# mlvlab/UP-NeRF

Hardware: AMD Instinct MI355X
Metric: training rays/sec (higher is better)
Workload: dtype f32 (f16x3 emulated: 3 fp16 MFMAs per product, fp32 accumulate); 1 GPU; BASELINE.json configs[1]: Brandenburg Gate shape, 4096 rays/GPU/step, 64 coarse + 128 fine samples, two 8x256 fields + candidate/colour heads + TransientNet + appearance/candidate embeddings (763 images), pose optimisation ON, full step incl. both Adam updates; rays_per_gpu=4096, n_images=763, N_samples=64, N_importance=128, parallelism=dp1, field=f16x3

## Files before the change

### include/upnerf_hip.h

```cpp
#ifndef UPNERF_HIP_H
#define UPNERF_HIP_H

#include <stdint.h>

#ifdef __cplusplus
extern "C" {
#endif

#define UPNERF_ABI_VERSION 11
#define UPNERF_EINVAL (-1)
#define UPNERF_EUNSUP (-2)

#ifndef UPNERF_TILE_ROWS
#define UPNERF_TILE_ROWS 64
#endif
#define UPNERF_X0 64
#define UPNERF_AUXK 80
#define UPNERF_CK 16
#define UPNERF_MAX_D 8

int upnerf_abi_version(void);

int upnerf_pose_rays_fwd(int R, const float* se3, const float* c2w, const float* dirs,
                         float* rays_o, float* rays_d, void* stream);
// ... 275 lines not shown
  int32_t planes;
  upnerf_wgrad_operand A, B;
  const int32_t* expo_a; const int32_t* expo_b;
  float* dW; float* db;
  int32_t ldo;
  int32_t n2;
  float* dW2; float* db2;
  int32_t ldo2, nsplit;
  const float* v; float* dv; float* dbv;
  float* slabs;
} upnerf_wgrad_desc;
long long upnerf_wgrad16_scratch(const upnerf_wgrad_desc* d);
int upnerf_wgrad16(const upnerf_wgrad_desc* d, upnerf_wgrad_pending* pending, void* stream);
int upnerf_wgrad_finish(upnerf_wgrad_pending* pending, void* stream);

int upnerf_vec_wgrad(int M, const float* v, int ldv, int nvec, const float* X, int ldx, int K,
                     float* dw , float* dbv , float* scratch, int nsplit, void* stream);

int upnerf_vec_wgrad_frag16(int M, const float* v, int ldv, int nvec, const uint16_t* X16, const int32_t* xexp, int K, float* dw,
                            float* dbv, float* scratch, int nsplit, void* stream);

int upnerf_ray_sum(int R, int S, const float* X, int C, float* out, void* stream);
int upnerf_ray_geom_bwd(int R, int S, const float* dxyz, const float* z, float* d_o, float* d_d, void* stream);

typedef struct {
  int32_t R, h, C;
  const int64_t* idx;
  const float* all_ray_infos;
  const float* all_directions;
  const float* all_rgbs;
// ... 539 lines not shown
```

### upnerf_amd/_lib.py

```python
from __future__ import annotations

import ctypes as C
import os

import torch

from .pass_plan import (AUXK, CK, RR_PART_STRIDE, TILE_PART_STRIDE, WG_F16_FRAG, WG_F16_TILE, WG_F24, WG_F32,
                        WG_PLANES, X0)

_HERE = os.path.dirname(os.path.abspath(__file__))
LIB_PATH = os.environ.get("UPNERF_LIB") or os.path.join(_HERE, "libupnerf_hip.so")
MAX_D = 8

_fp = C.c_void_p


class Layout(C.Structure):
    _fields_ = [("W", C.c_int32), ("D", C.c_int32), ("skip", C.c_int32),
                ("w", C.c_int32 * MAX_D), ("b", C.c_int32 * MAX_D),
                ("we", C.c_int32), ("be", C.c_int32), ("wsig", C.c_int32), ("bsig", C.c_int32),
                ("wc1", C.c_int32), ("bc1", C.c_int32), ("wc2", C.c_int32), ("bc2", C.c_int32),
                ("wcsig", C.c_int32), ("bcsig", C.c_int32), ("wr1", C.c_int32), ("br1", C.c_int32),
                ("wr2", C.c_int32), ("br2", C.c_int32), ("total", C.c_int32),
                ("t_w", C.c_int32 * MAX_D), ("t_skipx", C.c_int32), ("t_we", C.c_int32), ("t_head", C.c_int32),
# ... 93 lines not shown

class WgradPending(C.Structure):
    _fields_ = [("slabs", _fp), ("bslabs", _fp), ("dW", _fp), ("db", _fp), ("N", C.c_int32), ("K", C.c_int32), ("TN", C.c_int32),
                ("TK", C.c_int32), ("nsplit", C.c_int32), ("ldo", C.c_int32), ("rblocks", C.c_int32), ("n2", C.c_int32),
                ("dW2", _fp), ("db2", _fp), ("ldo2", C.c_int32), ("pad", C.c_int32), ("vslabs", _fp), ("dv", _fp), ("dbv", _fp)]


class WgradOperand(C.Structure):
    _fields_ = [("p", _fp), ("lo", _fp), ("exp", _fp), ("ld", C.c_int32), ("kind", C.c_int32)]


class WgradDesc(C.Structure):
    _fields_ = [("M", C.c_int32), ("N", C.c_int32), ("K", C.c_int32), ("planes", C.c_int32), ("A", WgradOperand), ("B", WgradOperand),
                ("expo_a", _fp), ("expo_b", _fp), ("dW", _fp), ("db", _fp), ("ldo", C.c_int32), ("n2", C.c_int32), ("dW2", _fp),
                ("db2", _fp), ("ldo2", C.c_int32), ("nsplit", C.c_int32), ("v", _fp), ("dv", _fp), ("dbv", _fp), ("slabs", _fp)]


class WgradGroup(C.Structure):
    _fields_ = [("A", _fp), ("B", _fp), ("dW", _fp), ("db", _fp), ("M", C.c_int32), ("N", C.c_int32), ("K", C.c_int32),
                ("lda", C.c_int32), ("ldb", C.c_int32), ("ldo", C.c_int32)]


MAX_WGRAD_GROUPS = 32


class EmbedGroup(C.Structure):
    _fields_ = [("g", _fp), ("out", _fp), ("dim", C.c_int32)]


class EmbedRowsGroup(C.Structure):
# ... 255 lines not shown
    "upnerf_sort_rows": [_i, _i, _p, _p],
    "upnerf_sample_coarse_keyed": [_i, _i, _p, _p, C.POINTER(Rng), _f, _i, _p, _p],
    "upnerf_resample_sort": [_i, _i, _p, _p, _i, _i, _p, _i, _p, _i, _i, _p, _i, _i, C.POINTER(Rng), _p, _p],
    "upnerf_ray_aux": [_i, _p, _p, C.POINTER(C.c_float), _p, _p, _p],
    "upnerf_field_fwd": [C.POINTER(Layout), C.POINTER(FieldFwdArgs), _p],
    "upnerf_composite_fwd": [C.POINTER(CompositeFwdArgs), _p],
    "upnerf_composite_bwd": [C.POINTER(CompositeBwdArgs), _p],
    "upnerf_field_bwd": [C.POINTER(Layout), C.POINTER(FieldBwdArgs), _p],
    "upnerf_field_fwd_f16x3": [C.POINTER(Layout), C.POINTER(FieldFwdArgs), _p],
    "upnerf_field_bwd_f16x3": [C.POINTER(Layout), C.POINTER(FieldBwdArgs), _p],
    "upnerf_frag16": [_p, _p, _p, C.POINTER(Frag16Desc), _i, C.POINTER(Frag16Desc), _i, _p, _p, _i, _i, _p, _p],
    "upnerf_wgrad": [_i, _p, _i, _i, _p, _i, _i, _p, _i, _p, _p, _i, _p],
    "upnerf_wgrad16_scratch": [C.POINTER(WgradDesc)],
    "upnerf_wgrad16": [C.POINTER(WgradDesc), C.POINTER(WgradPending), _p],
    "upnerf_wgrad_finish": [_p, _p],
    "upnerf_transient_fwd": [_p, _p],
    "upnerf_transient_bwd": [_p, _p, _p],
    "upnerf_wgrad_grouped_scratch": [C.POINTER(WgradGroup), _i, _i],
    "upnerf_wgrad_grouped": [C.POINTER(WgradGroup), _i, _p, _i, _p],
    "upnerf_vec_wgrad": [_i, _p, _i, _i, _p, _i, _i, _p, _p, _p, _i, _p],
    "upnerf_matvec": [_i, _i, _p, _i, _p, _p, _p, _i, _p],
    "upnerf_matvec_rank1": [_i, _i, _p, _i, _p, _p, _p, _i, _p, _p],
    "upnerf_add_pairs": [C.POINTER(AddPair), _i, _p],
    "upnerf_zero": [_p, C.c_longlong, _p],
    "upnerf_vec_wgrad_frag16": [_i, _p, _i, _i, _p, _p, _i, _p, _p, _p, _i, _p],
    "upnerf_ray_sum": [_i, _i, _p, _i, _p, _p],
    "upnerf_ray_part_finish": [_i, _i, _p, _p, _p, _p],
    "upnerf_tile_part_finish": [_i, _i, _p, _p, _p, _p, _p, _p, _p, _p, _p],
    "upnerf_ray_geom_bwd": [_i, _i, _p, _p, _p, _p, _p],
    "upnerf_pack": [_p, C.POINTER(PackDesc), _i, _i, _p],
# ... 48 lines not shown
    "upnerf_vit_embed": [_i, _i, _p, _p, _p, _p],
    "upnerf_layernorm": [_i, _i, _p, _i, _p, _p, _f, _p, _i, _p],
    "upnerf_vit_attention": [C.POINTER(VitAttentionArgs), _p],
    "upnerf_vit_gelu": [_p, C.c_longlong, _p],
    "upnerf_vit_residual": [_p, _p, C.c_longlong, _p],
    "upnerf_pca_fit_scratch": [_i, _i],
    "upnerf_pca_fit": [C.POINTER(PcaFitArgs), _p, _p],
    "upnerf_conv3x3": [C.POINTER(Conv3x3Args), _p],
    "upnerf_upsample2x": [C.POINTER(Upsample2xArgs), _p],
    "upnerf_depth_to_space": [C.POINTER(DepthToSpaceArgs), _p],
    "upnerf_resize_cubic": [C.POINTER(ResizeCubicArgs), _p],
    "upnerf_vit_patches16": [C.POINTER(VitPatches16Args), _p],
    "upnerf_baked_render": [C.POINTER(BakedRenderArgs), _p],
    "upnerf_baked_pack": [C.POINTER(BakedPackArgs), _p],
}
_LONGLONG = ("upnerf_wgrad16_scratch", "upnerf_mtet_scratch", "upnerf_occ_words", "upnerf_occ_build_scratch",
             "upnerf_occ_compact_scratch", "upnerf_pca_fit_scratch")
MAX_SCALARS = 96
EXPORTS = tuple(_SIGNATURES)


def _load():
    if not os.path.exists(LIB_PATH):
        raise ImportError(
            f"{LIB_PATH} not found: the HIP extension is not built. Run `python __graft_entry__.py` "
            "(there is no CPU/PyTorch fallback for the render_rays hot path).")
    lib = C.CDLL(LIB_PATH)
    for name, argtypes in _SIGNATURES.items():
        fn = getattr(lib, name, None)
        if fn is None:
            raise ImportError(f"{LIB_PATH} does not export {name}; rebuild it")
# ... 39 lines not shown
```

### upnerf_amd/csrc/wgrad_f16x3.hip

```cpp
#include "common.cuh"
#include "wgrad_host.h"

namespace {

typedef _Float16 h8 __attribute__((ext_vector_type(8)));
typedef _Float16 h4 __attribute__((ext_vector_type(4)));
typedef short s4 __attribute__((ext_vector_type(4)));
typedef unsigned int u32x2_t __attribute__((ext_vector_type(2)));

#ifndef FX_CHUNK_BIG
#define FX_CHUNK_BIG 16
#endif

template <int FX_CHUNK>
__device__ __forceinline__ int himg(int row, int col) {
  const int panel = col >> 7, c = col & 127;
  return panel * (FX_CHUNK * 256) + 256 * row + 16 * ((c >> 3) ^ (((row & 3) << 2) | ((row >> 2) & 3))) + 2 * (c & 7);
}

__device__ __forceinline__ h4 tr_read(const char* base, int byteoff) {
  s4 v = __builtin_amdgcn_ds_read_tr16_b64_v4i16((s4 __attribute__((address_space(3)))*)(base + byteoff));
  return __builtin_bit_cast(h4, v);
}

#define FX_THREADS 512
#define WG_LOAD(p) NT_LOAD(p)
#define WG_OPLOAD(dst, p) dst = WG_LOAD((const f32x4*)(p))
#define WG_PIN_LOADS_P __builtin_amdgcn_sched_barrier(0)
template <int NP, int MTW, int NTW, bool HASV = false>
__global__ __launch_bounds__(FX_THREADS, 1) void wgrad_f16x3_kernel(int M, int N, int K, const float* __restrict__ A, int lda,
                                                                  const float* __restrict__ B, int ldb,
                                                                  const int* __restrict__ expo_a, const int* __restrict__ expo_b,
                                                                  float* __restrict__ slabs, float* __restrict__ bslabs,
                                                                  int rows_per_split, upnerf_wgrad_pending prev,
                                                                  const float* __restrict__ vrow = nullptr,
                                                                  float* __restrict__ vslabs = nullptr) {
  constexpr int TN = 64 * MTW, TK = 64 * NTW;
  constexpr int FX_CHUNK = (MTW * NTW == 16) ? FX_CHUNK_BIG : 32;
  constexpr int PN = (TN + 127) / 128, PK = (TK + 127) / 128;
  constexpr int SZA = PN * FX_CHUNK * 256, SZB = PK * FX_CHUNK * 256;
  constexpr int A4 = FX_CHUNK * TN / 4 / FX_THREADS, B4 = FX_CHUNK * TK / 4 / FX_THREADS;
  static_assert(A4 >= 1 && B4 >= 1, "tile too small for 512 threads");
  constexpr int WK = (TK >= 128) ? 4 : 2, WN = 8 / WK;
  constexpr int MT = (TN / WN >= 32) ? TN / WN / 32 : 1, NT = TK / WK / 32;
  constexpr bool HALF = TN / WN < 32;
  __shared__ __attribute__((aligned(16))) char lds[2 * (2 * SZA + 2 * SZB)];
  const int tid = threadIdx.x, lane = tid & 63, wave = tid >> 6;
  const int li = lane & 31, hh = lane >> 5;
  const bool active = !HALF || wave < 4;
  const int wn = HALF ? ((wave & 3) >> 1) : wave / WK, wk = HALF ? (wave & 1) : wave % WK;
  const int n0 = wn * 32 * MT, k0 = wk * 32 * NT;
  const int split = blockIdx.x;
  const int nblk = blockIdx.y * TN, kblk = blockIdx.z * TK;
  const int mbeg = split * rows_per_split;
  const int mend = (mbeg + rows_per_split < M) ? mbeg + rows_per_split : M;
  if (prev.nsplit > 0) {
    const int wg = (blockIdx.z * gridDim.y + blockIdx.y) * gridDim.x + blockIdx.x;
    if (wg < prev.rblocks) {
      wgrad_reduce_body(wg, tid, prev, (f32x4(*)[64])lds);
      __syncthreads();
    }
  }
  const int ea = expo_a[0], eb = expo_b[0];
  const float sa = ldexpf(1.0f, ea), sb = ldexpf(1.0f, eb);

  f32x16 acc[MT][NT];
  acc_zero(acc);
  f32x4 bsum = {0.f, 0.f, 0.f, 0.f};

  f32x4 ra0[A4], rb0[B4], ra1[A4], rb1[B4];
  float rv0[B4], rv1[B4];
  f32x4 vsum = {0.f, 0.f, 0.f, 0.f};
  float vtot = 0.0f;
  const int mlast = mend > mbeg ? mend - 1 : (mbeg < M ? mbeg : M - 1);
  auto gload = [&](f32x4 (&ra)[A4], f32x4 (&rb)[B4], float (&rv)[B4], int mc) {
#pragma unroll
    for (int q = 0; q < A4; ++q) {
      const int idx = tid + q * FX_THREADS, row = idx / (TN / 4), c4 = idx - row * (TN / 4);
      const int m = mc + row < mlast ? mc + row : mlast;
      const int col = nblk + 4 * c4 < N ? nblk + 4 * c4 : 0;
      WG_OPLOAD(ra[q], &A[(size_t)m * lda + col]);
    }
#pragma unroll
    for (int q = 0; q < B4; ++q) {
      const int idx = tid + q * FX_THREADS, row = idx / (TK / 4), c4 = idx - row * (TK / 4);
      const int m = mc + row < mlast ? mc + row : mlast;
      const int col = kblk + 4 * c4 < K ? kblk + 4 * c4 : 0;
      WG_OPLOAD(rb[q], &B[(size_t)m * ldb + col]);
      if constexpr (HASV) rv[q] = vrow[m];
    }
  };
  auto split_store = [&](char* hi, char* lo, f32x4 v, float s, int row, int col) {
    typedef float f2 __attribute__((ext_vector_type(2)));
    typedef _Float16 hh2 __attribute__((ext_vector_type(2)));
    const f2 x0 = f2{v[0], v[1]} * s, x1 = f2{v[2], v[3]} * s;
    const hh2 h0 = __builtin_convertvector(x0, hh2), h1 = __builtin_convertvector(x1, hh2);
    const int off = himg<FX_CHUNK>(row, col);
    *(h4*)(hi + off) = __builtin_shufflevector(h0, h1, 0, 1, 2, 3);
    if constexpr (NP == 2) {
      const hh2 l0 = __builtin_convertvector(x0 - __builtin_convertvector(h0, f2), hh2);
      const hh2 l1 = __builtin_convertvector(x1 - __builtin_convertvector(h1, f2), hh2);
      *(h4*)(lo + off) = __builtin_shufflevector(l0, l1, 0, 1, 2, 3);
    }
  };
  auto lstore = [&](const f32x4 (&ra)[A4], const f32x4 (&rb)[B4], const float (&rv)[B4], int buf, int mc) {
    char* base = lds + buf * (2 * SZA + 2 * SZB);
    const f32x4 z4 = {0.f, 0.f, 0.f, 0.f};
#pragma unroll
    for (int q = 0; q < A4; ++q) {
      const int idx = tid + q * FX_THREADS, row = idx / (TN / 4), c4 = idx - row * (TN / 4);
      const f32x4 v = (mc + row < mend && nblk + 4 * c4 < N) ? ra[q] : z4;
      bsum += v;
      split_store(base, base + SZA, v, sa, row, 4 * c4);
    }
#pragma unroll
    for (int q = 0; q < B4; ++q) {
      const int idx = tid + q * FX_THREADS, row = idx / (TK / 4), c4 = idx - row * (TK / 4);
      const f32x4 v = (mc + row < mend && kblk + 4 * c4 < K) ? rb[q] : z4;
      split_store(base + 2 * SZA, base + 2 * SZA + SZB, v, sb, row, 4 * c4);
      if constexpr (HASV) {
        const float vm = mc + row < mend ? rv[q] : 0.0f;
        vsum += v * vm;
        vtot += c4 == 0 ? vm : 0.0f;
      }
    }
  };
  const int g = lane >> 4, tq = (lane >> 2) & 3, tp = lane & 3;
  const int trow = 8 * (g >> 1) + tq, tcol = 16 * (g & 1) + 4 * tp;

  auto contract = [&](int buf) {
    if (!active) return;
    const char* base = lds + buf * (2 * SZA + 2 * SZB);
#pragma unroll
    for (int kk = 0; kk < FX_CHUNK / 16; ++kk) {
      h8 ah[MT], al[MT];
#pragma unroll
      for (int mt = 0; mt < MT; ++mt) {
        const int o0 = himg<FX_CHUNK>(16 * kk + trow, n0 + 32 * mt + tcol), o1 = himg<FX_CHUNK>(16 * kk + trow + 4, n0 + 32 * mt + tcol);
        const h4 x0 = tr_read(base, o0), x1 = tr_read(base, o1);
        ah[mt] = __builtin_shufflevector(x0, x1, 0, 1, 2, 3, 4, 5, 6, 7);
        if constexpr (NP == 2) {
          const h4 y0 = tr_read(base + SZA, o0), y1 = tr_read(base + SZA, o1);
          al[mt] = __builtin_shufflevector(y0, y1, 0, 1, 2, 3, 4, 5, 6, 7);
        }
// ... 7 lines not shown
        if constexpr (NP == 2) {
          const h4 y0 = tr_read(base + 2 * SZA + SZB, o0), y1 = tr_read(base + 2 * SZA + SZB, o1);
          bl = __builtin_shufflevector(y0, y1, 0, 1, 2, 3, 4, 5, 6, 7);
        }
#pragma unroll
        for (int mt = 0; mt < MT; ++mt) {
          acc[mt][nt] = __builtin_amdgcn_mfma_f32_32x32x16_f16(ah[mt], bh, acc[mt][nt], 0, 0, 0);
          if constexpr (NP == 2) {
            acc[mt][nt] = __builtin_amdgcn_mfma_f32_32x32x16_f16(ah[mt], bl, acc[mt][nt], 0, 0, 0);
            acc[mt][nt] = __builtin_amdgcn_mfma_f32_32x32x16_f16(al[mt], bh, acc[mt][nt], 0, 0, 0);
          }
        }
      }
    }
  };
  constexpr bool TWO_SETS = MT * NT * 16 <= 64 || FX_CHUNK == 16;
  if constexpr (TWO_SETS) {
    gload(ra0, rb0, rv0, mbeg);
    gload(ra1, rb1, rv1, mbeg + FX_CHUNK);
#pragma unroll 1
    for (int mc = mbeg; mc < mend; mc += 2 * FX_CHUNK) {
      lstore(ra0, rb0, rv0, 0, mc);
      __syncthreads();
      gload(ra0, rb0, rv0, mc + 2 * FX_CHUNK);
      contract(0);
      lstore(ra1, rb1, rv1, 1, mc + FX_CHUNK);
      __syncthreads();
      gload(ra1, rb1, rv1, mc + 3 * FX_CHUNK);
      contract(1);
    }
  } else {
    int buf = 0;
    gload(ra0, rb0, rv0, mbeg);
#pragma unroll 1
    for (int mc = mbeg; mc < mend; mc += FX_CHUNK) {
      lstore(ra0, rb0, rv0, buf, mc);
      __syncthreads();
      gload(ra0, rb0, rv0, mc + FX_CHUNK);
      contract(buf);
      buf ^= 1;
    }
  }
  const float unscale = ldexpf(1.0f, -(ea + eb));
  const size_t blk = ((size_t)split * gridDim.y + blockIdx.y) * gridDim.z + blockIdx.z;
  float* slab = slabs + blk * TN * TK;
  if (active) {
#pragma unroll
    for (int mt = 0; mt < MT; ++mt)
#pragma unroll
      for (int nt = 0; nt < NT; ++nt)
#pragma unroll
        for (int r = 0; r < 16; ++r) {
          const int n = n0 + 32 * mt + (r & 3) + 8 * (r >> 2) + 4 * hh;
          slab[n * TK + k0 + 32 * nt + li] = acc[mt][nt][r] * unscale;
        }
  }
  if (bslabs && blockIdx.z == 0) {
    __syncthreads();
    f32x4* red = (f32x4*)lds;
    red[tid] = bsum;
    __syncthreads();
    constexpr int Q = TN / 4, G = FX_THREADS / Q;
    if (tid < Q) {
      f32x4 s = red[tid];
#pragma unroll
      for (int j = 1; j < G; ++j) s += red[tid + j * Q];
      *(f32x4*)&bslabs[((size_t)split * gridDim.y + blockIdx.y) * TN + 4 * tid] = s;
    }
  }
  if constexpr (HASV) {
// ... 623 lines not shown
  upnerf_wgrad_pending P = reduce_desc(d->N, d->K, TN, TK, nsplit, d->slabs, L.bslabs, d->dW, d->ldo, d->db);
  P.n2 = d->n2;
  P.dW2 = d->dW2;
  P.db2 = d->db2;
  P.ldo2 = d->ldo2;
  P.vslabs = L.vslabs;
  P.dv = d->dv;
  P.dbv = d->dbv;
  if (pending) {
    *pending = P;
    return 0;
  }
  launch_reduce(L.st, P);
  return (int)hipGetLastError();
}
```

### upnerf_amd/ops.py

```python
from __future__ import annotations

import contextlib
import ctypes as C
import os
from typing import Dict, NamedTuple, Optional, Tuple

import torch
import torch.nn.functional as F

from . import _lib
from ._lib import check, lib, ptr, stream

_WS: Dict[Tuple[str, int], torch.Tensor] = {}


class KernelTimer:

    def __init__(self):
        self.enabled = False
        self.only = None
        self.records = {}

    def run(self, name: str, fn, units: int = 0):
        if not self.enabled or (self.only is not None and name not in self.only):
# ... 148 lines not shown
        p = self.t.data_ptr() + 4 * self.off if self.kind == _lib.WG_F32 else ptr(self.t)
        return _lib.WgradOperand(p=p, lo=ptr(self.lo), exp=ptr(self.exp), ld=self.ld, kind=self.kind)


_WG_TIMER = {_lib.WG_F32: "wgrad16", _lib.WG_F16_TILE: "wgrad16p", _lib.WG_F16_FRAG: "wgrad16p", _lib.WG_F24: "wgrad24p",
             _lib.WG_PLANES: "wgrad16hl"}


class WgradRun:

    def __init__(self, device, chained: bool):
        self.device, self.pending, self.flip = device, _lib.WgradPending() if chained else None, 0

    def wgrad(self, M: int, A: WgOp, N: int, B: WgOp, K: int, expo_a: int, expo_b: int, *, dW: int, ldo: int, db: Optional[int] = None,
              n2: int = 0, dW2: Optional[int] = None, ldo2: int = 0, db2: Optional[int] = None, v: Optional[torch.Tensor] = None,
              dv: Optional[int] = None, dbv: Optional[int] = None, planes: int = 2):
        d = _lib.WgradDesc(M=M, N=N, K=K, planes=planes, A=A.c(), B=B.c(), expo_a=expo_a, expo_b=expo_b, dW=dW, db=db, ldo=ldo, n2=n2,
                           dW2=dW2, db2=db2, ldo2=ldo2, nsplit=nsplit_for(M), v=ptr(v), dv=dv, dbv=dbv)
        n = lib.upnerf_wgrad16_scratch(C.byref(d))
        if n < 0:
            check(n, "upnerf_wgrad16_scratch")
        if self.pending is None:
            tag = "wgrad"
        else:
            self.flip ^= 1
            tag = f"wgrad_chain{self.flip}"
        d.slabs = ptr(workspace(tag, n, self.device))
        pending = None if self.pending is None else C.byref(self.pending)
        check(TIMER.run(f"{_WG_TIMER[A.kind]}_{N}x{K}", lambda: lib.upnerf_wgrad16(C.byref(d), pending, stream()), units=M), "upnerf_wgrad16")

    def finish(self):
        if self.pending is not None:
            check(lib.upnerf_wgrad_finish(C.byref(self.pending), stream()), "upnerf_wgrad_finish")


def wgrad_f16x3_into(M: int, A: torch.Tensor, lda: int, N: int, B: torch.Tensor, ldb: int, K: int, dW_ptr: int, ldo: int,
                     db_ptr: Optional[int], device, expo: Optional[torch.Tensor] = None, expo_a: Optional[int] = None,
                     expo_b: Optional[int] = None, a_off: int = 0, b_off: int = 0, planes: int = 2):
    if expo_a is None:
        if expo is None:
            expo = scale_exponents(A, B)
        expo_a, expo_b = expo.data_ptr(), expo.data_ptr() + 4
    WgradRun(device, chained=False).wgrad(M, WgOp(A, lda, off=a_off), N, WgOp(B, ldb, off=b_off), K, expo_a, expo_b, dW=dW_ptr, ldo=ldo,
# ... 297 lines not shown
```

### upnerf_amd/pass_plan.py

```python
from __future__ import annotations

from collections import namedtuple
from functools import lru_cache
from itertools import accumulate

X0, AUXK, CK = 64, 80, 16
WG_F32, WG_F16_TILE, WG_F16_FRAG, WG_F24, WG_PLANES = range(5)
TILE_PART_STRIDE = 1288
RR_PART_STRIDE = 512
RR_TILE = 256
MODES = ("f16x3", "f32", "f16")

STAGES = {"aux": ("aux",),
          "field": ("sigma_s", "sigma_c", "rgb", "x0", "h16", "hexp", "h_lo8", "h", "e", "e16", "eexp", "hmask", "mx32", "g1", "g1_16",
                    "g1exp", "g2", "g2_16", "g2exp", "r1", "r1_16", "r1exp"),
          "composite": ("w_all", "w_sj", "w_cj", "w_s", "E_s", "G_c", "sum_sfeat", "t_weight", "c_depth", "s_depth", "rgb_map",
                        "rgb_joint_map"),
          "cbwd": ("d_sigma_s", "d_sigma_c", "d_rgb"),
          "fbwd": ("gz_e", "gz_h", "gz16", "gzexp", "gz_lo8", "gz_rg", "gz_rg16", "gzrgexp", "gz_g1", "gz_g2", "gz_g2_16", "gzg2exp",
                   "gz_r1", "dpre_s", "dpre_c", "dpre_rgb"),
          "part": ("tile_part", "ray_part"), "sums": ("rs_c", "rs_r")}
F16 = frozenset(("h16", "e16", "g1_16", "g2_16", "r1_16", "gz16", "gz_rg16", "gz_g2_16"))
I32 = frozenset(("hexp", "eexp", "g1exp", "g2exp", "r1exp", "gzexp", "gzrgexp", "gzg2exp"))
DTYPES = {**dict.fromkeys(F16, "float16"), **dict.fromkeys(I32, "int32"), "h_lo8": "uint8", "gz_lo8": "uint8", "hmask": "int64"}
# ... 205 lines not shown
        if joined:
            c.append(mat(("gz_rg", None), W, e, W, E.joined, E.final, L.wr1, wr1.ld, L.br1, n2=W2, dW2=L.wc1, ldo2=wc1.ld,
                         db2=L.bc1))
        else:
            c.append(mat(("gz_g1", None), W2, e, W, E.g1, E.final, L.wc1, wc1.ld, L.bc1))
        c.append(Launch(RAY, ("rs_c", None), ("c_rows", None), None, W2, CK, None, None, L.wc1 + wc1.part("c").col0, wc1.ld, None))
        c.append(mat(("gz_g2", None), W2, ("g1", None), W2, E.g2, E.g1, L.wc2, wc2.ld, L.bc2))
        c += [] if tile_part else [csig]
    if rgb:
        if not joined:
            r.append(mat(("gz_r1", None), W2, e, W, E.r1, E.final, L.wr1, wr1.ld, L.br1))
        r.append(Launch(RAY, ("rs_r", None), ("aux", None), None, W2, AUXK, None, None, L.wr1 + wr1.part("dir").col0, wr1.ld, None))
        r += [] if tile_part else [rgb2]
    part = (csig if cand else None, rgb2 if rgb else None) if tile_part else None
    return Schedule(tuple(trunk), part, tuple(c), tuple(r))
```

### upnerf_amd/rendering.py

```python
from __future__ import annotations

import ctypes as C
import os
from types import SimpleNamespace
from typing import Dict, List, Optional

import torch

from . import _lib, step_scalars, zero_pool
from ._lib import CompositeBwdArgs, CompositeFwdArgs, FieldBwdArgs, FieldFwdArgs, check, lib, ptr, stream
from .ops import (TIMER, WgOp, WgradRun, embed_rows, fanout, hip_linear, linear_kn_view, linear_raw, nsplit_for,
                  vec_wgrad_frag16_into, vec_wgrad_into, wgrad_into, workspace)
from .pass_plan import DTYPES, MAT, PADDED, RAY, RR_TILE, STAGES, VEC, VEC_FRAG, ZEROED, PassPlan, plan_pass, wgrad_schedule

__all__ = ["render_rays", "sample_pdf", "band_weights", "join_rays", "retain_ray_gradient", "ray_gradient"]


def _env_int(name: str, default: int) -> int:
    return int(os.environ.get("UPNERF_" + name, default))


FIELD_MODE = os.environ.get("UPNERF_FIELD_MODE", "f16x3")
WGRAD_STORE = os.environ.get("UPNERF_WGRAD_STORE", "f32")
TILE_PARTIALS = _env_int("TILE_PARTIALS", 1)
WGRAD_CHAIN = _env_int("WGRAD_CHAIN", 1)
VEC_RIDE = _env_int("VEC_RIDE", 1)
FUSE_RESAMPLE = _env_int("FUSE_RESAMPLE", 1)
JOIN_RAYS = _env_int("JOIN_RAYS", 1)
JOIN_HEADS = _env_int("JOIN_HEADS", 1)
FIELD_RR = _env_int("FIELD_RR", 1)
_SWITCHES = ("FIELD_MODE", "WGRAD_STORE", "FIELD_RR", "TILE_PARTIALS", "WGRAD_CHAIN", "JOIN_HEADS", "VEC_RIDE")


def _plan(pk, R: int, S: int, mode: int = 2, use_cand=False, use_rgb=False, rgb_joint=False, train=False) -> PassPlan:
    sw = {k: globals()[k] for k in _SWITCHES}
    return plan_pass(pk.W, pk.W2, pk.D, R, S, mode, bool(use_cand), bool(use_rgb), bool(rgb_joint), bool(train), **sw)


_PK256 = SimpleNamespace(W=256, W2=128, D=8)
_field16_ok = lambda pk, S: _plan(pk, 1, S).use16
_rr_ok = lambda S: S >= 32 and _plan(_PK256, 1, S).rr
_planes = lambda: _plan(_PK256, 1, 32).planes


_LINSPACE: Dict[tuple, torch.Tensor] = {}
# ... 151 lines not shown
        side_c, side_a = pk.block["wc1"].part("c"), pk.block["wr1"].part("a")
        if dP is not None:
            sched = wgrad_schedule(plan, pk.offsets, pk.skip, cfg.use_cand, cfg.use_rgb)
            at = lambda off: None if off is None else dP.data_ptr() + 4 * off
            e32 = torch.empty(32, device=dev, dtype=torch.int32)
            check(lib.upnerf_scale_exponents(ptr(sv["mx32"]), 32, ptr(e32), st), "upnerf_scale_exponents")
            run = WgradRun(dev, chained=WGRAD_CHAIN)
            held = {**sv, **bw}

            def op(name, l=None) -> WgOp:
                o = plan.operands[name]
                i = o.at if l is None else l
                pick = lambda k: None if k is None else held[k] if i is None else held[k][i]
                return WgOp(pick(o.data), o.ld, o.kind, pick(o.exp), pick(o.lo))

            def mat(r):
                head = {} if r.ride is None else dict(v=held[r.ride.v], dv=at(r.ride.dW), dbv=at(r.ride.db))
                run.wgrad(M, op(*r.A), r.N, op(*r.B), r.K, e32.data_ptr() + 4 * (16 + r.ea), e32.data_ptr() + 4 * r.eb, dW=at(r.dW),
                          ldo=r.ldo, db=at(r.db), n2=r.n2, dW2=at(r.dW2), ldo2=r.ldo2, db2=at(r.db2), planes=plan.planes, **head)

            def vec(r):
                v, X = held[r.v], op(*r.B)
                vec_wgrad_into(M, v, v.stride(0), r.N, X.t, X.ld, r.K, at(r.dW), at(r.db), dev)

            def vec_frag(r):
                v, X = held[r.v], op(*r.B)
                vec_wgrad_frag16_into(M, v, v.stride(0), r.N, X.t, X.exp, r.K, at(r.dW), at(r.db), dev)

            def ray(r):
                wgrad_into(R, bw[r.A[0]], r.N, r.N, sv[r.B[0]], r.K, r.K, at(r.dW), r.ldo, None, dev)
            execute = {MAT: mat, VEC: vec, VEC_FRAG: vec_frag, RAY: ray}

            def launch(segment):
                for r in segment:
                    execute[r.kind](r)
            launch(sched.trunk)
        bw.update(_alloc(plan, "sums", dev))
        rs_c, rs_r = bw["rs_c"], bw["rs_r"]
        if plan.partials == "tile":
            tgt = [at(o) for r in sched.part for o in ((r.dW, r.db) if r else (None, None))] if dP is not None else [None] * 4
            check(lib.upnerf_tile_part_finish(R, S, ptr(bw["tile_part"]), ptr(rs_c), ptr(rs_r), *tgt,
                                              ptr(workspace("tile_part", 128 * 520, dev)) if dP is not None else None, st),
                  "upnerf_tile_part_finish")
        elif plan.partials == "ray":
            check(lib.upnerf_ray_part_finish(R, S, ptr(bw["ray_part"]), ptr(rs_c), ptr(rs_r), st), "upnerf_ray_part_finish")
        if cfg.use_cand:
            if plan.partials == "none":
                check(lib.upnerf_ray_sum(R, S, ptr(gz_g1), W2, ptr(rs_c), st), "upnerf_ray_sum")
            if dP is not None:
                launch(sched.cand)
            if ctx.needs_input_grad[3]:
# ... 382 lines not shown
```

Baseline: 253,700 rays/s.

## Fuse skip-layer x0 weight-gradient into the 256x256 wgrad kernel as a riding operand

```diff
diff --git a/include/upnerf_hip.h b/include/upnerf_hip.h
--- a/include/upnerf_hip.h
+++ b/include/upnerf_hip.h
@@ -313,6 +313,15 @@
 int upnerf_wgrad16(const upnerf_wgrad_desc* d, upnerf_wgrad_pending* pending, void* stream);
 int upnerf_wgrad_finish(upnerf_wgrad_pending* pending, void* stream);
 
+typedef struct {
+  const float* B2;
+  const int32_t* expo_b2;
+  float* dW2x;
+  int32_t ldb2, K2, ldo2x, pad;
+} upnerf_wgrad_ride;
+long long upnerf_wgrad16_ride_scratch(const upnerf_wgrad_desc* d, const upnerf_wgrad_ride* ride);
+int upnerf_wgrad16_ride(const upnerf_wgrad_desc* d, const upnerf_wgrad_ride* ride, upnerf_wgrad_pending* pending, void* stream);
+
 int upnerf_vec_wgrad(int M, const float* v, int ldv, int nvec, const float* X, int ldx, int K,
                      float* dw , float* dbv , float* scratch, int nsplit, void* stream);
 
diff --git a/upnerf_amd/_lib.py b/upnerf_amd/_lib.py
--- a/upnerf_amd/_lib.py
+++ b/upnerf_amd/_lib.py
@@ -131,6 +131,11 @@
     _fields_ = [("M", C.c_int32), ("N", C.c_int32), ("K", C.c_int32), ("planes", C.c_int32), ("A", WgradOperand), ("B", WgradOperand),
                 ("expo_a", _fp), ("expo_b", _fp), ("dW", _fp), ("db", _fp), ("ldo", C.c_int32), ("n2", C.c_int32), ("dW2", _fp),
                 ("db2", _fp), ("ldo2", C.c_int32), ("nsplit", C.c_int32), ("v", _fp), ("dv", _fp), ("dbv", _fp), ("slabs", _fp)]
+
+
+class WgradRide(C.Structure):
+    _fields_ = [("B2", _fp), ("expo_b2", _fp), ("dW2x", _fp), ("ldb2", C.c_int32), ("K2", C.c_int32), ("ldo2x", C.c_int32),
+                ("pad", C.c_int32)]
 
 
 class WgradGroup(C.Structure):
@@ -416,6 +421,8 @@
     "upnerf_wgrad16_scratch": [C.POINTER(WgradDesc)],
     "upnerf_wgrad16": [C.POINTER(WgradDesc), C.POINTER(WgradPending), _p],
     "upnerf_wgrad_finish": [_p, _p],
+    "upnerf_wgrad16_ride_scratch": [C.POINTER(WgradDesc), C.POINTER(WgradRide)],
+    "upnerf_wgrad16_ride": [C.POINTER(WgradDesc), C.POINTER(WgradRide), C.POINTER(WgradPending), _p],
     "upnerf_transient_fwd": [_p, _p],
     "upnerf_transient_bwd": [_p, _p, _p],
     "upnerf_wgrad_grouped_scratch": [C.POINTER(WgradGroup), _i, _i],
@@ -494,7 +501,7 @@
     "upnerf_baked_render": [C.POINTER(BakedRenderArgs), _p],
     "upnerf_baked_pack": [C.POINTER(BakedPackArgs), _p],
 }
-_LONGLONG = ("upnerf_wgrad16_scratch", "upnerf_mtet_scratch", "upnerf_occ_words", "upnerf_occ_build_scratch",
+_LONGLONG = ("upnerf_wgrad16_scratch", "upnerf_wgrad16_ride_scratch", "upnerf_mtet_scratch", "upnerf_occ_words", "upnerf_occ_build_scratch",
              "upnerf_occ_compact_scratch", "upnerf_pca_fit_scratch")
 MAX_SCALARS = 96
 EXPORTS = tuple(_SIGNATURES)
diff --git a/upnerf_amd/csrc/wgrad_f16x3.hip b/upnerf_amd/csrc/wgrad_f16x3.hip
--- a/upnerf_amd/csrc/wgrad_f16x3.hip
+++ b/upnerf_amd/csrc/wgrad_f16x3.hip
@@ -27,16 +27,35 @@
 #define WG_LOAD(p) NT_LOAD(p)
 #define WG_OPLOAD(dst, p) dst = WG_LOAD((const f32x4*)(p))
 #define WG_PIN_LOADS_P __builtin_amdgcn_sched_barrier(0)
-template <int NP, int MTW, int NTW, bool HASV = false>
+struct wgrad_ride_args {
+  const float* B2;
+  const int* expo_b2;
+  int ldb2, K2;
+};
+typedef float f32x2v __attribute__((ext_vector_type(2)));
+typedef _Float16 h2v __attribute__((ext_vector_type(2)));
+#define FX_RIDE_K 64
+
+__device__ __forceinline__ wgrad_ride_args ride_of() { return wgrad_ride_args{}; }
+__device__ __forceinline__ wgrad_ride_args ride_of(const wgrad_ride_args& r) { return r; }
+
+template <int NP, int MTW, int NTW, bool HASV = false, class... RideArgs>
 __global__ __launch_bounds__(FX_THREADS, 1) void wgrad_f16x3_kernel(int M, int N, int K, const float* __restrict__ A, int lda,
                                                                   const float* __restrict__ B, int ldb,
                                                                   const int* __restrict__ expo_a, const int* __restrict__ expo_b,
                                                                   float* __restrict__ slabs, float* __restrict__ bslabs,
                                                                   int rows_per_split, upnerf_wgrad_pending prev,
                                                                   const float* __restrict__ vrow = nullptr,
-                                                                  float* __restrict__ vslabs = nullptr) {
+                                                                  float* __restrict__ vslabs = nullptr, RideArgs... ride_args) {
+  constexpr bool RIDE = sizeof...(RideArgs) == 1;
+  static_assert(sizeof...(RideArgs) <= 1, "at most one riding operand");
+  [[maybe_unused]] const wgrad_ride_args ride = ride_of(ride_args...);
   constexpr int TN = 64 * MTW, TK = 64 * NTW;
   constexpr int FX_CHUNK = (MTW * NTW == 16) ? FX_CHUNK_BIG : 32;
+  static_assert(!RIDE || (NP == 2 && MTW == 4 && NTW == 4 && !HASV), "the narrow operand rides on the 3-term 256 x 256 block");
+  constexpr int SZ2 = FX_CHUNK * 256;
+  constexpr int R2 = RIDE ? FX_CHUNK * FX_RIDE_K / 2 / FX_THREADS : 1;
+  static_assert(R2 >= 1, "riding panel too small for 512 threads");
   constexpr int PN = (TN + 127) / 128, PK = (TK + 127) / 128;
   constexpr int SZA = PN * FX_CHUNK * 256, SZB = PK * FX_CHUNK * 256;
   constexpr int A4 = FX_CHUNK * TN / 4 / FX_THREADS, B4 = FX_CHUNK * TK / 4 / FX_THREADS;
@@ -44,11 +63,13 @@
   constexpr int WK = (TK >= 128) ? 4 : 2, WN = 8 / WK;
   constexpr int MT = (TN / WN >= 32) ? TN / WN / 32 : 1, NT = TK / WK / 32;
   constexpr bool HALF = TN / WN < 32;
-  __shared__ __attribute__((aligned(16))) char lds[2 * (2 * SZA + 2 * SZB)];
+  constexpr int LDS_MAIN = 2 * (2 * SZA + 2 * SZB);
+  __shared__ __attribute__((aligned(16))) char lds[LDS_MAIN + (RIDE ? 2 * 2 * SZ2 : 0)];
   const int tid = threadIdx.x, lane = tid & 63, wave = tid >> 6;
   const int li = lane & 31, hh = lane >> 5;
   const bool active = !HALF || wave < 4;
   const int wn = HALF ? ((wave & 3) >> 1) : wave / WK, wk = HALF ? (wave & 1) : wave % WK;
+  const int wks = RIDE ? __builtin_amdgcn_readfirstlane(wk) : 0;
   const int n0 = wn * 32 * MT, k0 = wk * 32 * NT;
   const int split = blockIdx.x;
   const int nblk = blockIdx.y * TN, kblk = blockIdx.z * TK;
@@ -67,13 +88,25 @@
   f32x16 acc[MT][NT];
   acc_zero(acc);
   f32x4 bsum = {0.f, 0.f, 0.f, 0.f};
+  f32x16 acc2[2];
+  float sb2 = 0.0f;
+  int eb2 = 0;
+  if constexpr (RIDE) {
+#pragma unroll
+    for (int t = 0; t < 2; ++t)
+#pragma unroll
+      for (int r = 0; r < 16; ++r) acc2[t][r] = 0.0f;
+    eb2 = ride.expo_b2[0];
+    sb2 = ldexpf(1.0f, eb2);
+  }
 
   f32x4 ra0[A4], rb0[B4], ra1[A4], rb1[B4];
   float rv0[B4], rv1[B4];
+  f32x2v rc0[R2], rc1[R2];
   f32x4 vsum = {0.f, 0.f, 0.f, 0.f};
   float vtot = 0.0f;
   const int mlast = mend > mbeg ? mend - 1 : (mbeg < M ? mbeg : M - 1);
-  auto gload = [&](f32x4 (&ra)[A4], f32x4 (&rb)[B4], float (&rv)[B4], int mc) {
+  auto gload = [&](f32x4 (&ra)[A4], f32x4 (&rb)[B4], float (&rv)[B4], f32x2v (&rc)[R2], int mc) {
 #pragma unroll
     for (int q = 0; q < A4; ++q) {
       const int idx = tid + q * FX_THREADS, row = idx / (TN / 4), c4 = idx - row * (TN / 4);
@@ -88,6 +121,14 @@
       const int col = kblk + 4 * c4 < K ? kblk + 4 * c4 : 0;
       WG_OPLOAD(rb[q], &B[(size_t)m * ldb + col]);
       if constexpr (HASV) rv[q] = vrow[m];
+    }
+    if constexpr (RIDE) {
+#pragma unroll
+      for (int q = 0; q < R2; ++q) {
+        const int idx = tid + q * FX_THREADS, row = idx / (FX_RIDE_K / 2), c2 = idx - row * (FX_RIDE_K / 2);
+        const int m = mc + row < mlast ? mc + row : mlast;
+        rc[q] = WG_LOAD((const f32x2v*)&ride.B2[(size_t)m * ride.ldb2 + 2 * c2]);
+      }
     }
   };
   auto split_store = [&](char* hi, char* lo, f32x4 v, float s, int row, int col) {
@@ -103,7 +144,7 @@
       *(h4*)(lo + off) = __builtin_shufflevector(l0, l1, 0, 1, 2, 3);
     }
   };
-  auto lstore = [&](const f32x4 (&ra)[A4], const f32x4 (&rb)[B4], const float (&rv)[B4], int buf, int mc) {
+  auto lstore = [&](const f32x4 (&ra)[A4], const f32x4 (&rb)[B4], const float (&rv)[B4], const f32x2v (&rc)[R2], int buf, int mc) {
     char* base = lds + buf * (2 * SZA + 2 * SZB);
     const f32x4 z4 = {0.f, 0.f, 0.f, 0.f};
 #pragma unroll
@@ -124,10 +165,79 @@
         vtot += c4 == 0 ? vm : 0.0f;
       }
     }
+    if constexpr (RIDE) {
+      char* b2 = lds + LDS_MAIN + buf * (2 * SZ2);
+#pragma unroll
+      for (int q = 0; q < R2; ++q) {
+        const int idx = tid + q * FX_THREADS, row = idx / (FX_RIDE_K / 2), col = 2 * (idx - row * (FX_RIDE_K / 2));
+        const bool in = mc + row < mend;
+        const f32x2v x = f32x2v{(in && col < ride.K2) ? rc[q][0] : 0.0f, (in && col + 1 < ride.K2) ? rc[q][1] : 0.0f} * sb2;
+        const h2v h = __builtin_convertvector(x, h2v);
+        const int off = himg<FX_CHUNK>(row, col);
+        *(h2v*)(b2 + off) = h;
+        *(h2v*)(b2 + SZ2 + off) = __builtin_convertvector(x - __builtin_convertvector(h, f32x2v), h2v);
+      }
+    }
   };
   const int g = lane >> 4, tq = (lane >> 2) & 3, tp = lane & 3;
   const int trow = 8 * (g >> 1) + tq, tcol = 16 * (g & 1) + 4 * tp;
 
+#ifndef RIDE_MG
+#define RIDE_MG 1
+#endif
+  auto contract_ride = [&](int buf) {
+    static_assert(!RIDE || (MT == WK && MT % RIDE_MG == 0), "one n-tile of the riding panel per wave of an n-range");
+    const char* base = lds + buf * (2 * SZA + 2 * SZB);
+    const char* b2 = lds + LDS_MAIN + buf * (2 * SZ2);
+#pragma unroll
+    for (int kk = 0; kk < FX_CHUNK / 16; ++kk) {
+#pragma unroll
+      for (int g0 = 0; g0 < MT; g0 += RIDE_MG) {
+        __builtin_amdgcn_sched_barrier(0);
+        h8 ah[RIDE_MG], al[RIDE_MG];
+#pragma unroll
+        for (int j = 0; j < RIDE_MG; ++j) {
+          const int c = n0 + 32 * (g0 + j) + tcol;
+          const int o0 = himg<FX_CHUNK>(16 * kk + trow, c), o1 = himg<FX_CHUNK>(16 * kk + trow + 4, c);
+          const h4 x0 = tr_read(base, o0), x1 = tr_read(base, o1);
+          ah[j] = __builtin_shufflevector(x0, x1, 0, 1, 2, 3, 4, 5, 6, 7);
+          const h4 y0 = tr_read(base + SZA, o0), y1 = tr_read(base + SZA, o1);
+          al[j] = __builtin_shufflevector(y0, y1, 0, 1, 2, 3, 4, 5, 6, 7);
+        }
+#pragma unroll
+        for (int nt = 0; nt < NT; ++nt) {
+          const int o0 = himg<FX_CHUNK>(16 * kk + trow, k0 + 32 * nt + tcol), o1 = himg<FX_CHUNK>(16 * kk + trow + 4, k0 + 32 * nt + tcol);
+          const h4 x0 = tr_read(base + 2 * SZA, o0), x1 = tr_read(base + 2 * SZA, o1);
+          const h8 bh = __builtin_shufflevector(x0, x1, 0, 1, 2, 3, 4, 5, 6, 7);
+          const h4 y0 = tr_read(base + 2 * SZA + SZB, o0), y1 = tr_read(base + 2 * SZA + SZB, o1);
+          const h8 bl = __builtin_shufflevector(y0, y1, 0, 1, 2, 3, 4, 5, 6, 7);
+#pragma unroll
+          for (int j = 0; j < RIDE_MG; ++j) {
+            acc[g0 + j][nt] = __builtin_amdgcn_mfma_f32_32x32x16_f16(ah[j], bh, acc[g0 + j][nt], 0, 0, 0);
+            acc[g0 + j][nt] = __builtin_amdgcn_mfma_f32_32x32x16_f16(ah[j], bl, acc[g0 + j][nt], 0, 0, 0);
+            acc[g0 + j][nt] = __builtin_amdgcn_mfma_f32_32x32x16_f16(al[j], bh, acc[g0 + j][nt], 0, 0, 0);
+          }
+        }
+        if (wks >= g0 && wks < g0 + RIDE_MG) {
+#pragma unroll
+          for (int t = 0; t < 2; ++t) {
+            const int o0 = himg<FX_CHUNK>(16 * kk + trow, 32 * t + tcol), o1 = himg<FX_CHUNK>(16 * kk + trow + 4, 32 * t + tcol);
+            const h4 x0 = tr_read(b2, o0), x1 = tr_read(b2, o1);
+            const h8 bh = __builtin_shufflevector(x0, x1, 0, 1, 2, 3, 4, 5, 6, 7);
+            const h4 y0 = tr_read(b2 + SZ2, o0), y1 = tr_read(b2 + SZ2, o1);
+            const h8 bl = __builtin_shufflevector(y0, y1, 0, 1, 2, 3, 4, 5, 6, 7);
+#pragma unroll
+            for (int j = 0; j < RIDE_MG; ++j)
+              if (wks == g0 + j) {
+                acc2[t] = __builtin_amdgcn_mfma_f32_32x32x16_f16(ah[j], bh, acc2[t], 0, 0, 0);
+                acc2[t] = __builtin_amdgcn_mfma_f32_32x32x16_f16(ah[j], bl, acc2[t], 0, 0, 0);
+                acc2[t] = __builtin_amdgcn_mfma_f32_32x32x16_f16(al[j], bh, acc2[t], 0, 0, 0);
+              }
+          }
+        }
+      }
+    }
+  };
   auto contract = [&](int buf) {
     if (!active) return;
     const char* base = lds + buf * (2 * SZA + 2 * SZB);
@@ -165,46 +275,71 @@
       }
     }
   };
-  constexpr bool TWO_SETS = MT * NT * 16 <= 64 || FX_CHUNK == 16;
+  constexpr bool TWO_SETS = (MT * NT * 16 <= 64 || FX_CHUNK == 16) && !RIDE;
   if constexpr (TWO_SETS) {
-    gload(ra0, rb0, rv0, mbeg);
-    gload(ra1, rb1, rv1, mbeg + FX_CHUNK);
+    gload(ra0, rb0, rv0, rc0, mbeg);
+    gload(ra1, rb1, rv1, rc1, mbeg + FX_CHUNK);
 #pragma unroll 1
     for (int mc = mbeg; mc < mend; mc += 2 * FX_CHUNK) {
-      lstore(ra0, rb0, rv0, 0, mc);
+      lstore(ra0, rb0, rv0, rc0, 0, mc);
       __syncthreads();
-      gload(ra0, rb0, rv0, mc + 2 * FX_CHUNK);
+      gload(ra0, rb0, rv0, rc0, mc + 2 * FX_CHUNK);
       contract(0);
-      lstore(ra1, rb1, rv1, 1, mc + FX_CHUNK);
+      lstore(ra1, rb1, rv1, rc1, 1, mc + FX_CHUNK);
       __syncthreads();
-      gload(ra1, rb1, rv1, mc + 3 * FX_CHUNK);
+      gload(ra1, rb1, rv1, rc1, mc + 3 * FX_CHUNK);
       contract(1);
     }
   } else {
     int buf = 0;
-    gload(ra0, rb0, rv0, mbeg);
+    gload(ra0, rb0, rv0, rc0, mbeg);
 #pragma unroll 1
     for (int mc = mbeg; mc < mend; mc += FX_CHUNK) {
-      lstore(ra0, rb0, rv0, buf, mc);
+      lstore(ra0, rb0, rv0, rc0, buf, mc);
       __syncthreads();
-      gload(ra0, rb0, rv0, mc + FX_CHUNK);
-      contract(buf);
+      gload(ra0, rb0, rv0, rc0, mc + FX_CHUNK);
+      if constexpr (RIDE) contract_ride(buf);
+      else contract(buf);
       buf ^= 1;
     }
   }
   const float unscale = ldexpf(1.0f, -(ea + eb));
   const size_t blk = ((size_t)split * gridDim.y + blockIdx.y) * gridDim.z + blockIdx.z;
-  float* slab = slabs + blk * TN * TK;
-  if (active) {
+  constexpr int SP = RIDE ? FX_RIDE_K + TK : TK, SO = RIDE ? FX_RIDE_K : 0;
+  float* slab = slabs + blk * TN * SP;
+  if constexpr (!RIDE) {
+    if (active) {
+#pragma unroll
+      for (int mt = 0; mt < MT; ++mt)
+#pragma unroll
+        for (int nt = 0; nt < NT; ++nt)
+#pragma unroll
+          for (int r = 0; r < 16; ++r) {
+            const int n = n0 + 32 * mt + (r & 3) + 8 * (r >> 2) + 4 * hh;
+            slab[n * SP + SO + k0 + 32 * nt + li] = acc[mt][nt][r] * unscale;
+          }
+    }
+  } else {
+    int t2 = threadIdx.x;
+    asm volatile("" : "+v"(t2));
+    const int w2 = t2 >> 6, li2 = t2 & 31, hh2 = (t2 >> 5) & 1, wk2 = w2 % WK, n02 = (w2 / WK) * 32 * MT, k02 = wk2 * 32 * NT;
+    const float unscale2 = ldexpf(1.0f, -(ea + eb2));
 #pragma unroll
     for (int mt = 0; mt < MT; ++mt)
 #pragma unroll
       for (int nt = 0; nt < NT; ++nt)
 #pragma unroll
         for (int r = 0; r < 16; ++r) {
-          const int n = n0 + 32 * mt + (r & 3) + 8 * (r >> 2) + 4 * hh;
-          slab[n * TK + k0 + 32 * nt + li] = acc[mt][nt][r] * unscale;
-        }
+          const int n = n02 + 32 * mt + (r & 3) + 8 * (r >> 2) + 4 * hh2;
+          slab[n * SP + SO + k02 + 32 * nt + li2] = acc[mt][nt][r] * unscale;
+        }
+#pragma unroll
+    for (int t = 0; t < 2; ++t)
+#pragma unroll
+      for (int r = 0; r < 16; ++r) {
+        const int n = n02 + 32 * wk2 + (r & 3) + 8 * (r >> 2) + 4 * hh2;
+        slab[n * SP + 32 * t + li2] = acc2[t][r] * unscale2;
+      }
   }
   if (bslabs && blockIdx.z == 0) {
     __syncthreads();
@@ -858,3 +993,56 @@
   launch_reduce(L.st, P);
   return (int)hipGetLastError();
 }
+
+namespace {
+constexpr int RIDE_W = 256, RIDE_SP = RIDE_W + FX_RIDE_K;
+
+int check_ride(const upnerf_wgrad_desc* d, const upnerf_wgrad_ride* r) {
+  if (!d || !r) return UPNERF_EINVAL;
+  const int rc = check_desc(*d);
+  if (rc) return rc;
+  if (!r->B2 || !r->expo_b2 || !r->dW2x || r->K2 <= 0 || r->ldb2 <= 0 || (r->ldb2 & 3) || (r->ldo2x & 3)) return UPNERF_EINVAL;
+  if (d->A.kind != UPNERF_WG_F32 || d->B.kind != UPNERF_WG_F32 || d->planes == 1) return UPNERF_EUNSUP;
+  if (d->v || d->n2 > 0 || d->N != RIDE_W || d->K != RIDE_W || r->K2 > FX_RIDE_K) return UPNERF_EUNSUP;
+  if (r->ldb2 < FX_RIDE_K) return UPNERF_EINVAL;
+  if (r->dW2x + FX_RIDE_K != d->dW || r->ldo2x != d->ldo) return UPNERF_EUNSUP;
+  return 0;
+}
+}
+
+extern "C" long long upnerf_wgrad16_ride_scratch(const upnerf_wgrad_desc* d, const upnerf_wgrad_ride* r) {
+  if (!d || !r || d->nsplit <= 0) return UPNERF_EINVAL;
+  if (d->N != RIDE_W || d->K != RIDE_W || r->K2 <= 0 || r->K2 > FX_RIDE_K || d->v) return UPNERF_EUNSUP;
+  return (long long)d->nsplit * (RIDE_W * RIDE_SP + RIDE_W);
+}
+
+extern "C" int upnerf_wgrad16_ride(const upnerf_wgrad_desc* d, const upnerf_wgrad_ride* r, upnerf_wgrad_pending* pending, void* stream) {
+  int rc = check_ride(d, r);
+  if (rc) return rc;
+  if (pending && pending->nsplit > 0 && pending->slabs == d->slabs) return UPNERF_EINVAL;
+  const int nsplit = d->nsplit;
+  const int rows = (((d->M + nsplit - 1) / nsplit) + WG_CHUNK - 1) / WG_CHUNK * WG_CHUNK;
+  float* bslabs = d->slabs + (size_t)nsplit * RIDE_W * RIDE_SP;
+  upnerf_wgrad_pending prev = {};
+  if (pending && pending->nsplit > 0) {
+    if (pending->rblocks > nsplit) {
+      rc = upnerf_wgrad_finish(pending, stream);
+      if (rc) return rc;
+    } else {
+      prev = *pending;
+    }
+  }
+  hipLaunchKernelGGL((wgrad_f16x3_kernel<2, 4, 4, false, wgrad_ride_args>), dim3(nsplit, 1, 1), dim3(FX_THREADS), 0, (hipStream_t)stream,
+                     d->M, RIDE_W, RIDE_W, (const float*)d->A.p, d->A.ld, (const float*)d->B.p, d->B.ld, d->expo_a, d->expo_b, d->slabs,
+                     bslabs, rows, prev, (const float*)nullptr, (float*)nullptr,
+                     wgrad_ride_args{r->B2, r->expo_b2, r->ldb2, r->K2});
+  rc = (int)hipGetLastError();
+  if (rc) return rc;
+  const upnerf_wgrad_pending P = reduce_desc(RIDE_W, RIDE_SP, RIDE_W, RIDE_SP, nsplit, d->slabs, bslabs, r->dW2x, d->ldo, d->db);
+  if (pending) {
+    *pending = P;
+    return 0;
+  }
+  launch_reduce((hipStream_t)stream, P);
+  return (int)hipGetLastError();
+}
diff --git a/upnerf_amd/ops.py b/upnerf_amd/ops.py
--- a/upnerf_amd/ops.py
+++ b/upnerf_amd/ops.py
@@ -186,10 +186,14 @@
 
     def wgrad(self, M: int, A: WgOp, N: int, B: WgOp, K: int, expo_a: int, expo_b: int, *, dW: int, ldo: int, db: Optional[int] = None,
               n2: int = 0, dW2: Optional[int] = None, ldo2: int = 0, db2: Optional[int] = None, v: Optional[torch.Tensor] = None,
-              dv: Optional[int] = None, dbv: Optional[int] = None, planes: int = 2):
+              dv: Optional[int] = None, dbv: Optional[int] = None, planes: int = 2, ride2: Optional[tuple] = None):
         d = _lib.WgradDesc(M=M, N=N, K=K, planes=planes, A=A.c(), B=B.c(), expo_a=expo_a, expo_b=expo_b, dW=dW, db=db, ldo=ldo, n2=n2,
                            dW2=dW2, db2=db2, ldo2=ldo2, nsplit=nsplit_for(M), v=ptr(v), dv=dv, dbv=dbv)
-        n = lib.upnerf_wgrad16_scratch(C.byref(d))
+        r = None
+        if ride2 is not None:
+            B2, K2, expo_b2, dW2x = ride2
+            r = _lib.WgradRide(B2=B2.c().p, expo_b2=expo_b2, dW2x=dW2x, ldb2=B2.ld, K2=K2, ldo2x=ldo)
+        n = lib.upnerf_wgrad16_scratch(C.byref(d)) if r is None else lib.upnerf_wgrad16_ride_scratch(C.byref(d), C.byref(r))
         if n < 0:
             check(n, "upnerf_wgrad16_scratch")
         if self.pending is None:
@@ -199,6 +203,10 @@
             tag = f"wgrad_chain{self.flip}"
         d.slabs = ptr(workspace(tag, n, self.device))
         pending = None if self.pending is None else C.byref(self.pending)
+        if r is not None:
+            check(TIMER.run(f"{_WG_TIMER[A.kind]}_{N}x{K}+{K2}", lambda: lib.upnerf_wgrad16_ride(C.byref(d), C.byref(r), pending, stream()), units=M),
+                  "upnerf_wgrad16_ride")
+            return
         check(TIMER.run(f"{_WG_TIMER[A.kind]}_{N}x{K}", lambda: lib.upnerf_wgrad16(C.byref(d), pending, stream()), units=M), "upnerf_wgrad16")
 
     def finish(self):
diff --git a/upnerf_amd/pass_plan.py b/upnerf_amd/pass_plan.py
--- a/upnerf_amd/pass_plan.py
+++ b/upnerf_amd/pass_plan.py
@@ -243,3 +243,35 @@
         r += [] if tile_part else [rgb2]
     part = (csig if cand else None, rgb2 if rgb else None) if tile_part else None
     return Schedule(tuple(trunk), part, tuple(c), tuple(r))
+
+
+RIDE_K = 64
+
+
+def pair_skip(plan: PassPlan, trunk, planes=2):
+    ops = plan.operands
+
+    def rides(a, b):
+        return (a.kind == MAT and b.kind == MAT and a.A == b.A and a.B[0] == "x0" and b.B[0] == "h" and a.ride is None and b.ride is None
+                and plan.use16 and planes == 2 and all(ops[k].kind == WG_F32 for k in (a.A[0], "x0", "h"))
+                and a.N == b.N == 256 and b.K == 256 and a.K == RIDE_K and ops["x0"].ld >= RIDE_K and a.n2 == 0 and b.n2 == 0
+                and b.dW == a.dW + RIDE_K and a.ldo == b.ldo and b.db is None)
+
+    out, i = [], 0
+    while i < len(trunk):
+        if i + 1 < len(trunk) and rides(trunk[i], trunk[i + 1]):
+            out.append((trunk[i + 1]._replace(db=trunk[i].db), trunk[i]))
+            i += 2
+        else:
+            out.append((trunk[i], None))
+            i += 1
+    return tuple(out)
+
+
+def wgrad16_floats(N, K, nsplit, v=False, rider=False):
+    tile = lambda n: 256 if n >= 256 else 128 if n > 64 else 64
+    TN, TK = tile(N), tile(K)
+    gy, gz = -(-N // TN), -(-K // TK)
+    if rider:
+        return nsplit * (N * (RIDE_K + K) + N)
+    return nsplit * (gy * gz * TN * TK + gy * TN + (K + 4 if v else 0))
diff --git a/upnerf_amd/rendering.py b/upnerf_amd/rendering.py
--- a/upnerf_amd/rendering.py
+++ b/upnerf_amd/rendering.py
@@ -11,7 +11,8 @@
 from ._lib import CompositeBwdArgs, CompositeFwdArgs, FieldBwdArgs, FieldFwdArgs, check, lib, ptr, stream
 from .ops import (TIMER, WgOp, WgradRun, embed_rows, fanout, hip_linear, linear_kn_view, linear_raw, nsplit_for,
                   vec_wgrad_frag16_into, vec_wgrad_into, wgrad_into, workspace)
-from .pass_plan import DTYPES, MAT, PADDED, RAY, RR_TILE, STAGES, VEC, VEC_FRAG, ZEROED, PassPlan, plan_pass, wgrad_schedule
+from .pass_plan import (DTYPES, MAT, PADDED, RAY, RR_TILE, STAGES, VEC, VEC_FRAG, ZEROED, PassPlan, pair_skip, plan_pass,
+                        wgrad_schedule)
 
 __all__ = ["render_rays", "sample_pdf", "band_weights", "join_rays", "retain_ray_gradient", "ray_gradient"]
 
@@ -29,6 +30,7 @@
 JOIN_RAYS = _env_int("JOIN_RAYS", 1)
 JOIN_HEADS = _env_int("JOIN_HEADS", 1)
 FIELD_RR = _env_int("FIELD_RR", 1)
+SKIP_RIDE = True
 _SWITCHES = ("FIELD_MODE", "WGRAD_STORE", "FIELD_RR", "TILE_PARTIALS", "WGRAD_CHAIN", "JOIN_HEADS", "VEC_RIDE")
 
 
@@ -210,8 +212,10 @@
                 pick = lambda k: None if k is None else held[k] if i is None else held[k][i]
                 return WgOp(pick(o.data), o.ld, o.kind, pick(o.exp), pick(o.lo))
 
-            def mat(r):
+            def mat(r, rider=None):
                 head = {} if r.ride is None else dict(v=held[r.ride.v], dv=at(r.ride.dW), dbv=at(r.ride.db))
+                if rider is not None:
+                    head["ride2"] = (op(*rider.B), rider.K, e32.data_ptr() + 4 * rider.eb, at(rider.dW))
                 run.wgrad(M, op(*r.A), r.N, op(*r.B), r.K, e32.data_ptr() + 4 * (16 + r.ea), e32.data_ptr() + 4 * r.eb, dW=at(r.dW),
                           ldo=r.ldo, db=at(r.db), n2=r.n2, dW2=at(r.dW2), ldo2=r.ldo2, db2=at(r.db2), planes=plan.planes, **head)
 
@@ -230,7 +234,8 @@
             def launch(segment):
                 for r in segment:
                     execute[r.kind](r)
-            launch(sched.trunk)
+            for r, rider in pair_skip(plan, sched.trunk, plan.planes) if SKIP_RIDE else [(r, None) for r in sched.trunk]:
+                mat(r, rider) if rider is not None else execute[r.kind](r)
         bw.update(_alloc(plan, "sums", dev))
         rs_c, rs_r = bw["rs_c"], bw["rs_r"]
         if plan.partials == "tile":
```

New measurement: 255,100 rays/s (median of 6 runs). Within noise of the previous version (+0.6%).
